# EMI-Group/evogp

Hardware: AMD Instinct MI355X
Metric: tree_evals_per_s (higher is better)
Workload: dtype f32; 1 GPU; BASELINE north_star / configs[2] shape: SymbolicRegression synthetic 10-var, GLOBAL pop=1000000 x 1024 datapoints, max_tree_len=64, funcs + - * /, one tree_SR_fitness pass over every rank's shard per step; global_pop=1000000, pop_per_gpu=1000000, datapoints=1024, var_len=10, max_tree_len=64, ranks=1, device_prewarm_calls=40

## Files before the change

### evogp_amd/_lib.py

```python
from __future__ import annotations

import ctypes as C
import os

_HERE = os.path.dirname(os.path.abspath(__file__))
LIB_PATH = os.environ.get("EVOGP_HIP_LIB") or os.path.join(_HERE, "lib", "libevogp_hip.so")

ABI_VERSION = 9

_vp = C.c_void_p
_u = C.c_uint
_i = C.c_int
_f = C.c_float

PROTOTYPES = {
    "evogp_hip_generate": [_u, _u, _u, _u, _u, _f, _f, _vp, _vp, _vp, _vp, _vp, _vp, _vp, _u, _vp],
    "evogp_hip_mutate": [_i, _i, _vp, _vp, _vp, _vp, _vp, _vp, _vp, _vp, _vp, _vp, _vp],
    "evogp_hip_crossover": [_i, _i, _i, _vp, _vp, _vp, _vp, _vp, _vp, _vp, _vp, _vp, _vp, _vp],
    "evogp_hip_evaluate": [_u, _u, _u, _u, _vp, _vp, _vp, _vp, _vp, _vp],
    "evogp_hip_sr_fitness": [_u, _u, _u, _u, _u, _i, _vp, _vp, _vp, _vp, _vp, _vp, _u, _vp],
    "evogp_hip_generate_masked": [_u, _u, _u, _u, _u, _f, _f, _vp, _vp, _vp, _vp, _vp, _vp, _vp, _u, _vp, _u, _vp],
    "evogp_hip_breed_default": [_i, _i, _i, _i, _vp, _vp, _vp, _vp, _vp, _u, _vp, _vp, _vp, _vp, _vp, _vp, _vp, _vp],
    "evogp_hip_breed_default_rows": [_i, _i, _i, _i, _vp, _vp, _vp, _vp, _vp, _u, _vp, _vp, _vp, _vp, _vp, _vp, _vp, _i, _i, _vp],
    "evogp_hip_breed_default_table": [_i, _i, _i, _i, _i, _vp, _vp, _vp, _vp, _vp, _u, _vp, _vp, _vp, _vp, _vp, _vp, _vp, _i, _i, _vp],
    "evogp_hip_breed_lists": [_i, _i, _i, _i, _i, _vp, _vp, _vp, _vp, _vp, _vp, _u, _vp, _vp, _vp, _vp, _vp, _vp, _vp, _i, _i, _vp],
    "evogp_hip_generate_masked_hashed": [_u, _u, _u, _u, _u, _f, _f, _vp, _vp, _vp, _vp, _vp, _vp, _u, C.c_longlong, C.c_longlong, _u, _vp],
    "evogp_hip_breed_lists_hashed": [_i, _i, _i, _i, _i, _vp, _vp, _vp, _vp, _vp, C.c_longlong, C.c_longlong, _u, _vp, _vp, _vp, _vp, _vp, _vp, _vp, _i, _i, _vp],
    "evogp_hip_sr_fitness_hinted": [_u, _u, _u, _u, _u, _i, _vp, _vp, _vp, _vp, _vp, _vp, _u, _u, _vp],
    "evogp_hip_batch_evaluate": [_u, _u, _u, _u, _u, _vp, _vp, _vp, _vp, _vp, _vp],
    "evogp_hip_batch_argmax_count": [_u, _u, _u, _u, _u, _vp, _vp, _vp, _vp, _vp, _vp, _vp],
    "evogp_hip_evaluate_prepare": [_u, _u, _u, _u, _vp, _vp, _vp, _vp, C.c_size_t, _vp],
    "evogp_hip_evaluate_prepared": [_u, _u, _u, _u, _vp, _vp, _vp, _vp, _i, _vp, _vp, _vp],
    "evogp_hip_structural_mutate": [_i, _i, _i, _f, _i, _i, _i, C.c_longlong, C.c_longlong, _vp, _vp, _vp, _vp, _vp, _vp, _vp, _vp],
    "evogp_hip_insert_mutate": [_i, _i, C.c_uint, _i, C.c_longlong, C.c_longlong, _vp, _vp, _vp, _vp, _vp, _vp, _vp, _vp, _vp, _vp, _vp],
    "evogp_hip_point_mutate": [_i, _i, _i, _f, _f, _i, _i, _i, _i, _i, _i, _i, C.c_longlong, C.c_longlong, _vp, _vp, _vp, _vp, _vp, _vp, _vp, _vp, _vp],
    "evogp_hip_random_words": [C.c_longlong, C.c_longlong, _i, C.c_longlong, C.c_longlong, C.c_longlong, _vp, _vp],
    "evogp_hip_fitness_scores": [_u, _i, _vp, _vp, _vp],
    "evogp_hip_select": [_u, _u, _u, _vp, _vp, _vp, _vp],
    "evogp_hip_select_alternating": [_u, _u, _u, _vp, _vp, _vp, _vp, _vp],
    "evogp_hip_tournament_select": [_u, _u, _u, C.c_longlong, C.c_longlong, _vp, _vp, _vp],
    "evogp_hip_set_program_buffer_limit": [C.c_ulonglong],
    "evogp_hip_release_workspaces": [],
    "evogp_hip_set_allocator": [_vp, _vp],
    "evogp_hip_set_sr_division": [C.c_int],
    "evogp_hip_get_sr_division": [],
    "evogp_hip_abi_version": [],
    "evogp_hip_sr_gradient": [_u, _u, _u, _u, _u, _i, _vp, _vp, _vp, _vp, _vp, _vp, _vp, _vp],
    "evogp_hip_sr_const_step": [_u, _u, _u, _i, _vp, _vp, _vp, _vp, _vp, _vp, _vp, _vp, _vp, _vp],
    "evogp_hip_sr_case_errors": [_u, _u, _u, _u, _u, _i, _vp, _vp, _vp, _vp, _vp, _vp, _vp],
    "evogp_hip_lexicase_workspace_bytes": [_u, _u, _u, C.POINTER(C.c_ulonglong)],
    "evogp_hip_lexicase_select": [_u, _u, _vp, _vp, _u, C.c_longlong, C.c_longlong, _vp, _vp, _vp],
    "evogp_hip_pareto_rank_workspace_bytes": [_u, C.POINTER(C.c_ulonglong)],
    "evogp_hip_pareto_rank": [_u, _u, _vp, _vp, _vp, _vp, _vp, _vp, _vp],
    "evogp_hip_nsga2_select": [_u, _vp, _u, _u, _u, C.c_longlong, C.c_longlong, _vp, _vp],
    "evogp_hip_sr_subtree_errors": [_u, _u, _u, _u, _u, _i, _vp, _vp, _vp, _vp, _vp, _vp, _vp, _vp],
    "evogp_hip_prune_rows": [_u, _u, _u, _i, _i, _vp, _vp, _vp, _vp, _vp, _vp, _vp, _vp, _vp, _vp, _vp],
}

DEBUG_PROTOTYPES = {
    "evogp_hip_timer_begin": [_vp],
    "evogp_hip_timer_end": [_vp, C.POINTER(C.c_float)],
    "evogp_hip_debug_set_stats": [_vp],
    "evogp_hip_debug_compile_batch": [_i],
    "evogp_hip_debug_long_compiler": [_i],
    "evogp_hip_debug_twins": [_i],
    "evogp_hip_debug_tc_fold": [_i],
    "evogp_hip_debug_profile": [_i],
    "evogp_hip_debug_profile_read": [C.POINTER(C.c_float), C.POINTER(C.c_int)],
    "evogp_hip_debug_tc_histogram": [_u, _vp, _i, _vp],
    "evogp_hip_debug_tc_nhandlers": [],
    "evogp_hip_debug_tc_program": [_u, _vp, _i],
    "evogp_hip_debug_forget_function_classes": [],
    "evogp_hip_debug_structural_mutate_given": [_i, _i, _i, _i, _i, _vp, _vp, _vp, _vp, _vp, _vp, _vp, _vp],
    "evogp_hip_debug_insert_mutate_given": [_i, _i, _i, _vp, _vp, _vp, _vp, _vp, _vp, _vp, _vp, _vp, _vp, _vp],
    "evogp_hip_debug_point_mutate_given": [_i, _i, _i, _i, _i, _i, _i, _i, _i, _vp, _vp, _vp, _vp, _vp, _vp, _vp, _vp, _vp, _vp, _vp, _vp, _vp, _vp],
    "evogp_hip_debug_lexicase": [_vp, _i],
    "evogp_hip_debug_pareto_rank": [_i],
}


def _load() -> C.CDLL:
    if not os.path.exists(LIB_PATH):
        raise ImportError(
            f"{LIB_PATH} is missing: build the HIP engine first "
            "(python -c 'import __graft_entry__ as g; g.build()'  or  make -C evogp_amd/csrc). "
            "evogp_amd has no CPU fallback."
        )
    lib = C.CDLL(LIB_PATH)
    for name, argtypes in list(PROTOTYPES.items()) + list(DEBUG_PROTOTYPES.items()):
        fn = getattr(lib, name)
        fn.argtypes = argtypes
        fn.restype = _i
    lib.evogp_hip_evaluate_workspace_bytes.argtypes = [_u, _u]
    lib.evogp_hip_evaluate_workspace_bytes.restype = C.c_size_t
    lib.evogp_hip_select_workspace_bytes.argtypes = []
    lib.evogp_hip_select_workspace_bytes.restype = C.c_size_t
    lib.evogp_hip_program_buffer_bytes.argtypes = []
    lib.evogp_hip_program_buffer_bytes.restype = C.c_ulonglong
    lib.evogp_hip_record_ring_bytes.argtypes = []
    lib.evogp_hip_record_ring_bytes.restype = C.c_ulonglong
    lib.evogp_hip_error_string.argtypes = [_i]
    lib.evogp_hip_error_string.restype = C.c_char_p
    got = lib.evogp_hip_abi_version()
    if got != ABI_VERSION:
        raise ImportError(f"libevogp_hip.so ABI version {got}, expected {ABI_VERSION}: rebuild the engine")
    return lib


lib = _load()


def check(code: int, what: str) -> None:
    if code != 0:
        raise RuntimeError(f"{what} failed: {lib.evogp_hip_error_string(code).decode()} (code {code})")
```

### evogp_amd/csrc/sr_tc.hip

```cpp
#include "interp.hpp"
#include "launch.hpp"
#include "sr_params.hpp"
#include "tc_interp_k8.inc"
#include "tc_interp_k4.inc"
#include "tc_interp_k1.inc"

#include <atomic>
#include <cstddef>
#include <mutex>
#include <cstdio>
#include <vector>

namespace evogp {

struct TcCompileParams {
    const float *value;
    const int16_t *type;
    const int16_t *size;
    uint2 *prog;
    float *fitness;
    unsigned *marks;
    unsigned *zero_next;
    int pop, gp_len, var_len;
    uint32_t unary_mask;
    uint32_t var_stride;
    uint32_t ydelta;
    uint32_t rec;
    uint32_t overflow;
    int depth;
    int out_len;
    int nblocks;
    int rows;
    int general;
    int heavy_reserve;
    int div_reserve;
    int classify;
    uint32_t recip;
    int twins;
    int long_fast;
    int learn;
    int nan_trees;
};

__device__ inline uint32_t division_in_place(uint32_t id, int after, const TcCompileParams &p) {
    if (id < 24u || id >= 32u) return id;
    const uint32_t form = id - 24u;
    const uint32_t ip = form == 0u ? (uint32_t)EVOGP_TC_H_DIVIP_SS : form == 3u ? (uint32_t)EVOGP_TC_H_DIVIP_SC : form == 4u ? (uint32_t)EVOGP_TC_H_DIVIP_CS : 0u;
    if (ip == 0u) return id;
    const int before = after + (form == 0u ? 1 : 0);
    return before + p.div_reserve <= p.depth ? ip : id;
}

enum : int { TC_S = 0, TC_V = 1, TC_C = 2 };
constexpr int kMarkSampleBlocks = 64;
constexpr int kZeroRounds = 3;
static std::atomic<int> g_long_fast{-1};
static std::atomic<int> g_twins{-1};
static std::atomic<int> g_fold{-1};
static std::atomic<int> g_compile_batch{-2};
static int tc_nan_trees() {
    static const int env_fold = env_int("EVOGP_TC_FOLD", 2);
    const int fo = g_fold.load(std::memory_order_relaxed);
    return fo >= 0 ? fo : (env_fold < 0 || env_fold > 2 ? 2 : env_fold);
}
static_assert(kSentinelHeavy == 0x7FC0FEEDu, "gen/gen_tc_asm.py SENTINEL_HEAVY");

__device__ inline float fold_bin4_fast(int op, float x, float y) {
    return op == 0 ? x + y : op == 1 ? x - y : op == 2 ? x * y : (y == 0.0f ? __builtin_nanf("") : x / y);
}

__device__ inline uint32_t tc_word0(int id, int slot, uint32_t pf_bytes, uint32_t aux = 0u) {
    return ((pf_bytes >> 10) << 24) | ((aux & 0xFFu) << 16) | (uint32_t)(((slot & 1) * EVOGP_TC_NHANDLERS + id) * EVOGP_TC_SLOT);
}

static_assert(EVOGP_TC_H_PUSH_V == EVOGP_TC_H_PUSH_C + 1 && EVOGP_TC_H_DIVIP_CS == EVOGP_TC_H_DIVIP_SS + 2 && EVOGP_TC_H_DIVR_CV == EVOGP_TC_H_DIVR_SV + 2 &&
              EVOGP_TC_H_PUSH_C_NP == EVOGP_TC_H_ADD_SS_NP + 24 && EVOGP_TC_H_DIVIP_SS_NP == EVOGP_TC_H_ADD_SS_NP + 26 &&
              EVOGP_TC_H_DIVR_SV_NP == EVOGP_TC_H_ADD_SS_NP + 29, "gen/gen_tc_asm.py NOPF_TWINS");
__device__ inline int no_prefetch_delta(bool arith3, bool push_c, bool in_place, bool by_recip) {
    return arith3 ? (int)EVOGP_TC_H_ADD_SS_NP : push_c ? (int)EVOGP_TC_H_PUSH_C_NP - (int)EVOGP_TC_H_PUSH_C
         : in_place ? (int)EVOGP_TC_H_DIVIP_SS_NP - (int)EVOGP_TC_H_DIVIP_SS : by_recip ? (int)EVOGP_TC_H_DIVR_SV_NP - (int)EVOGP_TC_H_DIVR_SV : 0;
}
__device__ inline bool next_word_has_variable(const TcCompileParams &, unsigned long long keptwave, bool kept, bool uses_var, bool is_root) {
    const unsigned long long U = __ballot(kept & uses_var);
    return __builtin_amdgcn_inverse_ballot_w64((((~keptwave) + (U << 1)) & keptwave) | __ballot(is_root));
}

__device__ inline void division_by_reciprocal(const TcCompileParams &p, int &id, uint32_t pf, uint32_t d1, uint32_t &aux) {
    const bool sv = id == 3 * 8 + 1, vv = id == 3 * 8 + 5, cv = id == 3 * 8 + 7;
    const bool ok = (p.recip != 0u) & (sv | vv | cv);
    const uint32_t voff = vv ? d1 << 4 : pf;
    aux = ok ? (voff + p.recip) >> 10 : aux;
    id = ok ? (int)EVOGP_TC_H_DIVR_SV + (int)vv + 2 * (int)cv : id;
}

constexpr int kUnaryInv = 10;
constexpr int kUnaryZero = 11;
__device__ __attribute__((always_inline)) inline float fold_unary_body(int op, float x) {
    switch (op) {
    case 0: return -x;
    case 1: return fabsf(x);
    case 2: return sinf(x);
    case 3: return cosf(x);
    case 4: return tanf(x);
    case 5: return sqrtf(x);
    case 6: return sqrtf(fabsf(x));
    case 7: return expf(x);
    case 8: return logf(x);
    case 9: return x == 0.0f ? -kMaxVal : logf(fabsf(x));
    case kUnaryZero: return 0.0f;
    default: return x == 0.0f ? __builtin_nanf("") : 1.0f / x;
    }
}
__device__ __attribute__((noinline)) float fold_unary(int op, float x) { return fold_unary_body(op, x); }

template <bool UN>
__device__ inline int compile_tree(const TcCompileParams &p, uint2 *rec, int len, int ty, int sz, float val, int lane) {
// ... 334 lines not shown
            int z = seli(L(Z0), 1, 0);
            int zr = bperm(z, ri4);
#pragma unroll
            for (int r = 0; r < kZeroRounds; ++r) {
                z |= (next(z) & ((zr & zboth) | zleft)) | (zr & zright);
                zr = bperm(z, ri4);
            }
            Mnan |= Mfn & Mop3 & B(zr != 0);
        }
    }
    const int nanincl = (int)__builtin_amdgcn_mbcnt_hi((uint32_t)(Mnan >> 32), __builtin_amdgcn_mbcnt_lo((uint32_t)Mnan, 0u)) + seli(L(Mnan), 1, 0);
    const int both = (int)((uint32_t)inclf << 15) | (nanincl << 8) | above;
    const int at_end = bperm(both, (end - 1) << 2), before = bperm(both, (lo - 1) << 2);
    const int base = seli(lo > 0, before >> 15, 0);
    const int slot = above - (at_end & 0xFF);
    const int totf = (at_end >> 15) - base;
    const int hf = seli(L(Mkept), totf - (inclf - base - deltaf), 0);
    M Mpz = Min & B(((at_end >> 8) & 127) != seli(lo > 0, (before >> 8) & 127, 0));
    if (U0 && Mpz != 0ull) {
        const M segmask = L(Min) ? ((len >= 64 ? ~0ull : ((1ull << len) - 1ull)) << lo) : 0ull;
        Mpz &= B((MU & segmask) == 0ull);
    }
    const M Mhigh = B(hf > p.depth);
    M Mlong = 0ull;
    if (U0) Mlong = Mroot & B(slot + 1 > 31);
    int cls = TREE_OK;
    if ((Min & (~(Mleaf | M4) | Msb | Mhigh | Mlong)) != 0ull) {
        const M segmask = L(Min) ? ((len >= 64 ? ~0ull : ((1ull << len) - 1ull)) << lo) : 0ull;
        auto seg_any = [&](M m) -> bool { return (m & segmask) != 0ull; };
        cls = seg_any(Min & B(kind == 3)) ? TREE_HEAVY : seg_any(Min & B(kind == 5)) ? TREE_GENERAL : seg_any(Min & Msb) ? TREE_HEAVY
            : seg_any(Min & Mhigh) ? (p.gp_len > 64 && p.general ? TREE_GENERAL : TREE_HEAVY) : seg_any(Mlong) ? TREE_HEAVY : TREE_OK;
    }
    const M Mdivown = MB & ~Mpushc & ~Mdivr & B(opx == 3);
    const M Mss = Mdivown & B(form == 0), Msc = Mdivown & B(form == 3), Mcs = Mdivown & B(form == 4);
    const int ip = seli(L(Mss), (int)EVOGP_TC_H_DIVIP_SS, seli(L(Msc), (int)EVOGP_TC_H_DIVIP_SC, (int)EVOGP_TC_H_DIVIP_CS));
    const M Minpl = (Mss | Msc | Mcs) & B(hf + seli(L(Mss), 1, 0) + p.div_reserve <= p.depth);
    id = seli(L(Minpl), ip, id);
    if (p.twins) {
        const M Muses = ~Mpushc & ~MU & ((MB & (MlV | MrV)) | (~MB & MV));
        const M Uk = Mkept & Muses;
        const M nxt = (((~keptwave) + (Uk << 1)) & keptwave) | Mroot;
        id += seli(L(nxt), 0, no_prefetch_delta(L(MB & ~Mpushc & ~Mdivr & B(opx < 3)), L(Mpushc), L(Minpl), L(Mdivr & ~Mpushc)));
    }
    const M Mok = B(cls == TREE_OK);
    if (L(Mkept & Mok & ~Mpz)) *(uint2 *)(rec0 + (roff + (uint32_t)slot * 8u)) = make_uint2(tc_word0(id, slot, pf, aux), d1);
    if (L(Mroot)) {
        uint32_t skip = tc_word0(EVOGP_TC_H_SKIP, 0, 0u), nan_tree = tc_word0(EVOGP_TC_H_NAN_TREE, 0, 0u);
        asm volatile("" : "+v"(skip), "+v"(nan_tree));
        const uint32_t last = selu(L(Mpz), nan_tree, tc_word0(EVOGP_TC_H_END, slot + 1, p.ydelta));
        *(uint2 *)(rec0 + (roff + (uint32_t)seli(L(Mok & ~Mpz), slot + 1, 0) * 8u)) = make_uint2(selu(L(Mok), last, skip), 0u);
    }
    if (cls == TREE_GENERAL && !p.general) cls = TREE_HEAVY;
    return L(Min) ? cls : (int)TREE_OK;
}

template <bool U0>
__device__ inline int compile_pack_arith_plain(const TcCompileParams &p, char *rec0, uint32_t roff, bool in, int lo, int len, int ty, int sz, float val, int lane) {
    auto bperm = [](int v, int i4) -> int { return __builtin_amdgcn_ds_bpermute(i4, v); };
    auto next = [](int v) -> int { return __builtin_amdgcn_update_dpp(0, v, 0x130 , 0xf, 0xf, true); };
    auto any = [](bool c) -> bool { return __builtin_amdgcn_ballot_w64(c) != 0ull; };
    auto seli = [](bool c, int x, int y) -> int { return c ? x : y; };
    auto selu = [](bool c, uint32_t x, uint32_t y) -> uint32_t { return c ? x : y; };
    auto self = [](bool c, float x, float y) -> float { return c ? x : y; };
    const int end = lo + len;
    const uint32_t f = (uint32_t)val;
    const bool isV = ty == T_VAR, isC = ty == T_CONST, isBf = ty == T_BFUNC;
    const uint32_t opu = f - (uint32_t)F_ADD;
    const bool is4 = isBf & (opu < 4u);
    const bool g5 = (isBf & (f - (uint32_t)F_LOOSE_DIV <= (uint32_t)(F_GE - F_LOOSE_DIV))) | (ty == T_TFUNC) | (ty == T_UFUNC);
    const int v = max(0, min((int)val, p.var_len - 1));
    const uint32_t pay = selu(isV, (uint32_t)v * p.var_stride, f2bits(val));
    const bool u0 = U0 && in & (ty == T_UFUNC) & (f - (uint32_t)F_SIN > (uint32_t)(F_LOOSE_SQRT - F_SIN)) & (p.unary_mask != 0u);
    const int kind = seli(isV, 0, seli(isC, 1, seli(is4, 2, seli(u0, 4, seli(g5, 5, 3)))));
    const int op = (int)(opu & 3u);
    const bool isB = in & (kind == 2), isU = U0 && u0;
    const int ks = kind | (sz << 3);
    const int ksl = next(ks);
    const int szl = ksl >> 3;
    const int ri = lane + 1 + szl, ri4 = ri << 2;
    const int ksr = bperm(ks, ri4);
    const int szr = ksr >> 3;
    const bool size_bad = (sz != seli(isB, 1 + szl + szr, seli(isU, 1 + szl, 1))) | (isB & ((szl < 1) | (ri >= end))) | (isU & ((szl < 1) | (lane + 1 >= end)));
    int kl = ksl & 7, kr = ksr & 7;
    uint32_t pl = (uint32_t)next((int)pay), pr = (uint32_t)bperm((int)pay, ri4);
    auto fold = [&](uint32_t a, uint32_t b, bool who) -> uint32_t {
        const float x = bits2f(a), y = bits2f(b);
        const float fa = x + y, fs = x - y, fm = x * y;
        float fd = fm;
        if (any(who & (op == 3))) fd = self(y == 0.0f, __builtin_nanf(""), x / y);
        return f2bits(self(op == 0, fa, self(op == 1, fs, self(op == 2, fm, fd))));
    };
    const bool absorbedB = isB & (kl == 1) & (kr == 1);
    const bool absorbed = absorbedB | (isU & (kl == 1));
    uint32_t folded = 0u;
    if (any(absorbed)) {
        folded = selu(absorbedB, fold(pl, pr, absorbedB), 0u);
        const int ek = seli(absorbed, 1, kind);
        const uint32_t ep = selu(absorbed, folded, pay);
        kl = next(ek); kr = bperm(ek, ri4);
        pl = (uint32_t)next((int)ep); pr = (uint32_t)bperm((int)ep, ri4);
    }
    if (U0) { kl = seli(kl == 4, 2, kl); kr = seli(kr == 4, 2, kr); }
    const bool cc = isB & !absorbed & (kl == 1) & (kr == 1);
    uint32_t folded2 = 0u;
    if (any(cc)) folded2 = fold(pl, pr, cc);
    const uint32_t cb = pr & 0x7FFFFFFFu, ex = cb >> 23;
// ... 1045 lines not shown
        else if (len <= 64) {
            if (__any(lane < len && ty == T_UFUNC && p.unary_mask != 0u)) cls = compile_tree<true>(p, rec, len, ty, sz, val, lane);
            else cls = compile_tree_arith(p, rec, len, ty, sz, val, lane);
        }
        if (cls == TREE_GENERAL && !p.general) cls = TREE_HEAVY;
        if (cls != TREE_OK && lane == 0) {
            rec[0] = make_uint2(tc_word0(EVOGP_TC_H_SKIP, 0, 0u), 0u);
            p.fitness[t] = cls == TREE_BAD ? __builtin_nanf("") : bits2f(cls == TREE_GENERAL ? kSentinelGeneral : kSentinelHeavy);
            if (cls == TREE_GENERAL && p.marks) p.marks[4] = 1u;
            else if (cls == TREE_HEAVY && p.marks) {
                p.marks[0] = 1u;
                if (blockIdx.x < kMarkSampleBlocks) atomicAdd(p.marks + 2, 1u);
            }
        }
    }
}

__device__ inline bool generic_node(int ty, float val) {
    const uint32_t f = (uint32_t)val;
    return (ty == T_TFUNC) | ((ty == T_BFUNC) & (f - (uint32_t)F_ADD >= 4u)) | ((ty == T_UFUNC) & ((f == (uint32_t)F_LOOSE_INV) | (f - (uint32_t)F_SINH <= 2u)));
}

template <int B, int MODE, bool LONGROWS>
__global__ __launch_bounds__(256) void tc_compile_packed_kernel(TcCompileParams p) {
    constexpr bool UN = MODE != 0;
    const int lane = threadIdx.x & 63;
    if (p.zero_next && blockIdx.x == 0)
        for (int i = threadIdx.x; i < kCallScratchWords; i += blockDim.x) p.zero_next[i] = 0u;
    const uint32_t wave_id = uni((blockIdx.x * blockDim.x + threadIdx.x) >> 6);
    const uint32_t t0 = wave_id * (uint32_t)B;
    if (t0 >= (uint32_t)p.pop) return;
    const int nb = (int)min((uint32_t)B, (uint32_t)p.pop - t0);
    const int L = p.gp_len;
    int raw = 1;
    if (lane < nb) raw = (int)p.size[(size_t)(t0 + (uint32_t)lane) * L];
    char *const rec0 = (char *)p.prog + (size_t)t0 * p.rec;
    const bool longer = LONGROWS && lane < nb && min(raw, L) > 64;
    if (LONGROWS && longer) {
        uint32_t skip = tc_word0(EVOGP_TC_H_SKIP, 0, 0u);
        asm volatile("" : "+v"(skip));
        *(uint2 *)(rec0 + (uint32_t)__mul24(lane, (int)p.rec)) = make_uint2(skip, 0u);
        p.fitness[t0 + (uint32_t)lane] = bits2f(p.general ? kSentinelGeneral : kSentinelHeavy);
        if (p.marks) {
            if (p.general) {
                const int n = min(raw, L);
                p.marks[p.long_fast ? 8 + (int)(n > 128) + (int)(n > 256) + (int)(n > 512) : 4] = 1u;
            }
            else {
                p.marks[0] = 1u;
                if ((wave_id >> 2) < (uint32_t)kMarkSampleBlocks) atomicAdd(p.marks + 2, 1u);
            }
        }
    }
    const int lens = lane < nb && !longer ? max(1, min(raw, L)) : 0;
    int sval = lens | (raw <= 0 ? 128 : 0) | (lane << 8);
#pragma unroll
    for (int r = 3; r < 7; ++r) {
        const unsigned long long ones = __builtin_amdgcn_ballot_w64((sval & (1 << r)) != 0);
        const int below1 = (int)__builtin_amdgcn_mbcnt_hi((uint32_t)(ones >> 32), __builtin_amdgcn_mbcnt_lo((uint32_t)ones, 0u));
        const int to = (sval & (1 << r)) ? below1 : __popcll(ones) + lane - below1;
        sval = __builtin_amdgcn_ds_permute(to << 2, sval);
    }
    const int slen = sval & 127;
    const size_t node0 = (size_t)t0 * (uint32_t)L;
    const float *const value0 = p.value + node0;
    const int16_t *const type0 = p.type + node0, *const size0 = p.size + node0;
    unsigned long long left = LONGROWS ? __builtin_amdgcn_ballot_w64(slen > 0) : (nb >= 64 ? ~0ull : (1ull << nb) - 1ull);
    bool n_in = false;
    unsigned long long n_inm = 0ull;
    int n_tb = 0, n_lo = 0, n_len = 0, n_bad = 0, n_ty = T_CONST, n_sz = 1;
    float n_val = 0.0f;
    auto plan = [&]() {
        int used = 0, about = 0;
        while (true) {
            const unsigned long long cand = __builtin_amdgcn_ballot_w64(slen <= 64 - used) & left;
            if (cand == 0ull) break;
            const int j = __builtin_ctzll(cand);
            left &= ~(1ull << j);
            const int sv = __builtin_amdgcn_readlane(sval, j), l = sv & 127;
            about = (uint32_t)(lane - used) < (uint32_t)l ? (sv | (used << 16)) : about;
            used += l;
            if (used >= 64) break;
        }
        n_in = lane < used;
        n_inm = used >= 64 ? ~0ull : (1ull << used) - 1ull;
        n_tb = (about >> 8) & 255; n_lo = about >> 16; n_len = about & 127; n_bad = about & 128;
        n_ty = T_CONST; n_sz = 1; n_val = 0.0f;
        if (n_in) {
            const uint32_t at = (uint32_t)(__mul24(n_tb, L) + lane - n_lo);
            n_ty = (int)*(const int16_t *)((const char *)type0 + at * 2u); n_val = *(const float *)((const char *)value0 + at * 4u);
            n_sz = (int)*(const int16_t *)((const char *)size0 + at * 2u);
        }
    };
    bool more = left != 0ull;
    if (more) plan();
    uint32_t seen = 0u;
    while (more) {
        const bool in = n_in;
        const unsigned long long inm = n_inm;
        const int tb = n_tb, lo = n_lo, len = n_len, bad = n_bad, sz = n_sz;
        const int ty = bad ? -1 : n_ty;
        const float val = n_val;
        more = left != 0ull;
        if (more) plan();
        const uint32_t roff = (uint32_t)__mul24(tb, (int)p.rec);
        int cls;
        const bool unary = __builtin_amdgcn_ballot_w64(ty == T_UFUNC) != 0ull;
        if (MODE == 3) cls = compile_pack_mo(p, rec0, roff, in, lo, len, ty, sz, val, lane);
        else if (MODE == 2 && __builtin_amdgcn_ballot_w64(generic_node(ty, val)) != 0ull) cls = compile_pack_generic(p, rec0, roff, in, lo, len, ty, sz, val, lane);
        else if (UN && unary && p.unary_mask != 0u) cls = compile_pack_unary<true>(p, rec0, roff, in, lo, len, ty, sz, val, lane);
        else if (!UN && unary) cls = compile_pack_arith<true>(p, rec0, roff, inm, lo, len, ty, sz, val, lane);
        else cls = compile_pack_arith<false>(p, rec0, roff, inm, lo, len, ty, sz, val, lane);
        if (MODE != 3 && p.learn) {
            const bool look = MODE != 0 || __builtin_amdgcn_ballot_w64(cls != TREE_OK) != 0ull;
            if (look) {
                const bool gen = __builtin_amdgcn_ballot_w64(generic_node(ty, val)) != 0ull;
                const bool un = unary && __builtin_amdgcn_ballot_w64((ty == T_UFUNC) & ((uint32_t)val - (uint32_t)F_SIN <= (uint32_t)(F_LOOSE_SQRT - F_SIN))) != 0ull;
                seen |= ((un | gen) ? 1u : 0u) | (gen ? 2u : 0u);
            }
        }
        if (cls != TREE_OK && in && lane == lo) {
            const bool nan = bad != 0 || cls == TREE_BAD;
            p.fitness[t0 + (uint32_t)tb] = nan ? __builtin_nanf("") : bits2f(cls == TREE_GENERAL ? kSentinelGeneral : kSentinelHeavy);
            if (!nan && p.marks) {
                if (cls == TREE_GENERAL) p.marks[p.long_fast ? 8 : 4] = 1u;
                else {
                    p.marks[0] = 1u;
                    if ((wave_id >> 2) < (uint32_t)kMarkSampleBlocks) atomicAdd(p.marks + 2, 1u);
                }
            }
        }
    }
    if (MODE != 3 && p.learn && p.marks && uni((int)seen) != 0 && lane == 0) {
        p.marks[5] = 1u;
        if (seen & 2u) p.marks[6] = 1u;
    }
}


__device__ __attribute__((always_inline)) inline int compile_long_arith(const TcCompileParams &p, char *rec0, int t, int len, char *lds, int lane,
                                                           int ty0, float val0, int sz0, int ty1, float val1, int sz1, int lds_len) {
    auto any = [](bool c) -> bool { return __builtin_amdgcn_ballot_w64(c) != 0ull; };
    auto seli = [](bool c, int x, int y) -> int { return c ? x : y; };
    auto selu = [](bool c, uint32_t x, uint32_t y) -> uint32_t { return c ? x : y; };
    const int L = lds_len;
    uint32_t *ks_s = (uint32_t *)lds;
// ... 886 lines not shown
        }
        records = (char *)d.prog;
    }
    if (!d.last_use && (e = hipEventCreateWithFlags(&d.last_use, hipEventDisableTiming)) != hipSuccess) return e;
    d.last_pop = p.pop; d.last_rec = rec; d.last_overflow = (uint32_t)overflow;

    int chunks = 1;
    static const int env_chunks = env_int("EVOGP_TC_CHUNKS", 0);
    if (p.marks && !capturing && !STATS && !p.prof_mid && pieces == 1) {
        if (env_chunks > 0) chunks = env_chunks;
        if (chunks > kCallScratchChunks) chunks = kCallScratchChunks;
        if (chunks > 1 && p.pop / chunks < 20000) chunks = p.pop / 20000 > 0 ? p.pop / 20000 : 1;
    }
    if (chunks > 1) {
        if (!d.side && (e = hipStreamCreateWithFlags(&d.side, hipStreamNonBlocking)) != hipSuccess) return e;
        if (!d.fork && (e = hipEventCreateWithFlags(&d.fork, hipEventDisableTiming)) != hipSuccess) return e;
        for (int i = 0; i < chunks; ++i)
            if (!d.ready[i] && (e = hipEventCreateWithFlags(&d.ready[i], hipEventDisableTiming)) != hipSuccess) return e;
        if (wg_waves * 2 > waves_per_cu) wg_waves = waves_per_cu / 2 > 0 ? waves_per_cu / 2 : 1;
        wgs_per_cu = 1;
    }
    *mark_sample = 0;
    static const int env_general = env_int("EVOGP_TC_GENERAL", 1);
    static const int env_unary = env_int("EVOGP_TC_UNARY", EVOGP_TC_UNARY_MASK | (1 << kUnaryInv));
    static const int env_cblocks = env_int("EVOGP_TC_CBLOCKS", 0);
    static const int env_divip = env_int("EVOGP_TC_DIVIP", 1);
    static const int env_long_fast = env_int("EVOGP_TC_LONG_FAST", 1);
    if (p.out_len > 1 && env_general == 0) return hipSuccess;

    auto compile_params = [&](int lo, int n, unsigned *marks, bool first) -> TcCompileParams {
        TcCompileParams c{};
        c.value = p.value + (size_t)lo * p.gp_len; c.type = p.type + (size_t)lo * p.gp_len; c.size = p.size + (size_t)lo * p.gp_len;
        c.prog = (uint2 *)(records + (size_t)lo * rec); c.fitness = p.fitness + lo; c.marks = marks;
        c.zero_next = first ? p.zero_next : nullptr;
        c.pop = n; c.gp_len = p.gp_len; c.var_len = p.var_len;
        c.var_stride = (uint32_t)(tiles * G * 1024);
        c.ydelta = c.var_stride * (uint32_t)p.var_len;
        c.rec = rec; c.depth = DEPTH; c.overflow = (uint32_t)overflow;
        c.out_len = p.out_len; c.nblocks = nblocks; c.rows = K;
        c.heavy_reserve = (EVOGP_TC_HEAVY_REGS + K - 1) / K;
        c.div_reserve = env_divip ? (EVOGP_TC_DIVIP_REGS + K - 1) / K : 1 << 20;
        c.classify = p.classify;
        c.recip = recip ? (uint32_t)(p.var_len + label_cols) * c.var_stride : 0u;
        {
            static const int env_twins = env_int("EVOGP_TC_TWINS", 1);
            const int tw = g_twins.load(std::memory_order_relaxed);
            c.twins = tw >= 0 ? tw : (env_twins == 2 || (env_twins == 1 && (long)n >= 900l * info.num_cus));
        }
        c.general = env_general != 0;
        { const int lf = g_long_fast.load(std::memory_order_relaxed); c.long_fast = (lf >= 0 ? lf : env_long_fast) && p.out_len == 1 && p.gp_len >= 128 && c.general; }
        c.unary_mask = (uint32_t)env_unary & ((uint32_t)EVOGP_TC_UNARY_MASK | (1u << kUnaryInv));
        c.learn = p.feedback != nullptr && marks != nullptr;
        c.nan_trees = tc_nan_trees();
        return c;
    };
    bool learn_packed = false;
    auto launch_marked_general = [&](const TcCompileParams &c, int n, hipStream_t strm) {
        long gblocks = ((long)n + 63) / 64;
        if (gblocks > (long)info.num_cus * 16) gblocks = (long)info.num_cus * 16;
        if (p.gp_len <= 64) { hipLaunchKernelGGL(tc_compile_general_kernel<false>, dim3((unsigned)gblocks), dim3(256), 0, strm, c, 0, 0, p.gp_len); return; }
        if (c.long_fast && c.general && c.gp_len >= 128) {
            if (4 * tc_long_lds_bytes(c.gp_len) > 64 * 1024 && !d.attr_set[16]) {
                (void)hipFuncSetAttribute((const void *)tc_compile_long_kernel, hipFuncAttributeMaxDynamicSharedMemorySize, 160 * 1024 - 1024);
                (void)hipGetLastError();
                d.attr_set[16] = true;
            }
            int lo_len = 0, klass = 0;
            for (int hi_len = 128; ; hi_len *= 2, ++klass) {
                if (hi_len > c.gp_len) hi_len = c.gp_len;
                const int group = hi_len <= 256 ? 16 : 64;
                hipLaunchKernelGGL(tc_compile_long_kernel, dim3((unsigned)((n + group - 1) / group)), dim3(256), 4 * tc_long_lds_bytes(hi_len), strm, c, lo_len, hi_len, group, klass);
                if (hi_len >= c.gp_len) break;
                lo_len = hi_len;
            }
        }
        hipLaunchKernelGGL(tc_compile_general_kernel<true>, dim3((unsigned)gblocks), dim3(256), 4 * tc_general_lds_bytes(p.gp_len), strm, c, 0, 0, p.gp_len);
    };
    auto launch_compilers = [&](int lo, int n, unsigned *marks, bool first, hipStream_t strm) -> hipError_t {
        const TcCompileParams c = compile_params(lo, n, marks, first);
        long cblocks = ((long)n + 3) / 4;
        long cmax = (long)info.num_cus * 32;
        if (env_cblocks > 0) cmax = env_cblocks;
        if (cblocks > cmax) cblocks = cmax;
        if (first) {
            const long nwaves = cblocks * 4, sw = kMarkSampleBlocks * 4 < nwaves ? kMarkSampleBlocks * 4 : nwaves;
            long sample = 0;
            for (long w = 0; w < sw && w < n; ++w) sample += (n - 1 - w) / nwaves + 1;
            *mark_sample = (int)sample;
        }
        const size_t clds = 4 * tc_general_lds_bytes(p.gp_len);
        if (clds > 64 * 1024 && !d.attr_set[15]) {
            (void)hipFuncSetAttribute((const void *)tc_compile_general_kernel<true>, hipFuncAttributeMaxDynamicSharedMemorySize, 160 * 1024 - 1024);
            (void)hipGetLastError();
            d.attr_set[15] = true;
        }
        static const int env_packed_env = env_int("EVOGP_TC_PACKED", -1);
        const int set_packed = g_compile_batch.load(std::memory_order_relaxed);
        const int env_packed = set_packed != -2 ? set_packed : env_packed_env;
        static const int env_generic = env_int("EVOGP_TC_PACK_GENERIC", 1);
        const bool packed_mo = p.out_len > 1 && env_packed != 0 && env_generic != 0;
        const bool packed = (p.out_len == 1 && env_packed != 0) || packed_mo;
        if (packed) {
            const bool un = c.nblocks != 1;
            constexpr unsigned kOwnHandlers = (1u << F_ADD) | (1u << F_SUB) | (1u << F_MUL) | (1u << F_DIV) | (1u << F_SIN) | (1u << F_COS) | (1u << F_TAN) |
                                              (1u << F_LOG) | (1u << F_LOOSE_LOG) | (1u << F_EXP) | (1u << F_INV) | (1u << F_NEG) | (1u << F_ABS) |
                                              (1u << F_SQRT) | (1u << F_LOOSE_SQRT);
// ... 439 lines not shown
    if (p.out_len > 1 && p.out_len + 3 > EVOGP_TC_K8_DEPTH && k == 8) {
        if (env_wide && p.out_len + 3 <= EVOGP_TC_K8W_DEPTH && !p.stats) wide = true; else k = 4;
    }
    if (p.out_len > 1 && p.out_len + 3 > EVOGP_TC_K4_DEPTH && k == 4) return hipSuccess;
    if (p.out_len > 1 && p.out_len + 3 > EVOGP_TC_K1_DEPTH) return hipSuccess;
    static const int env_k = env_int("EVOGP_TC_K", 0);
    if (env_k == 1 || env_k == 4 || env_k == 8) k = env_k;
#ifndef EVOGP_FUSED_STATS
    if (p.stats) return run_tc<8, true>(p, stream, handled, mark_sample, mark_chunks);
#endif
    const int dm = sr_division_mode();
#ifdef EVOGP_FUSED_STATS
    static const int env_fused = env_int("EVOGP_TC_FUSED", 1);
#else
    static const int env_fused = env_int("EVOGP_TC_FUSED", -1);
#endif
    const bool fused_ok = k == 8 && p.out_len == 1 && !p.classify && p.gp_len <= 64 && p.marks && !p.prof_mid;
    auto fused = [&]() -> hipError_t {
        return dm == 1 ? run_fused<1>(p, stream, handled, mark_sample, mark_chunks)
             : dm == 2 ? run_fused<2>(p, stream, handled, mark_sample, mark_chunks)
                       : run_fused<0>(p, stream, handled, mark_sample, mark_chunks);
    };
    if (env_fused == 1 && fused_ok && !p.hint_general) {
        hipError_t fe = fused();
        if (fe != hipSuccess || *handled) return fe;
    }
#define EVOGP_RUN_TC(F) (wide && k == 8 ? run_tc<8, false, F, true>(p, stream, handled, mark_sample, mark_chunks) \
                        : k == 8 ? run_tc<8, false, F>(p, stream, handled, mark_sample, mark_chunks) \
                        : k == 4 ? run_tc<4, false, F>(p, stream, handled, mark_sample, mark_chunks) \
                                 : run_tc<1, false, F>(p, stream, handled, mark_sample, mark_chunks))
    hipError_t te = dm == 1 ? EVOGP_RUN_TC(1) : dm == 2 ? EVOGP_RUN_TC(2) : EVOGP_RUN_TC(0);
#undef EVOGP_RUN_TC
    if (te == hipSuccess && *handled && env_fused != 0 && fused_ok) fused_keep_spare(stream);
    if (te != hipSuccess || *handled || env_fused == 0 || !fused_ok) return te;
    if (g_prog_limit.load(std::memory_order_relaxed) == 0ull) return te;
    *mark_sample = 0; *mark_chunks = 1;
    return fused();
}

}

extern "C" int evogp_hip_debug_twins(int mode) {
    if (mode < -1 || mode > 1) return EVOGP_E_BADARG;
    evogp::g_twins.store(mode, std::memory_order_relaxed);
    return EVOGP_OK;
}

extern "C" int evogp_hip_debug_tc_fold(int mode) {
    if (mode < -1 || mode > 2) return EVOGP_E_BADARG;
    evogp::g_fold.store(mode, std::memory_order_relaxed);
    return EVOGP_OK;
}

extern "C" int evogp_hip_debug_long_compiler(int fast) {
    if (fast < -1 || fast > 1) return EVOGP_E_BADARG;
    evogp::g_long_fast.store(fast, std::memory_order_relaxed);
    return EVOGP_OK;
}

extern "C" int evogp_hip_debug_compile_batch(int trees) {
    if (trees < -1 || trees > 64) return EVOGP_E_BADARG;
    evogp::g_compile_batch.store(trees, std::memory_order_relaxed);
    return EVOGP_OK;
}

extern "C" int evogp_hip_set_program_buffer_limit(unsigned long long bytes) {
    evogp::g_prog_limit.store(bytes, std::memory_order_relaxed);
    return EVOGP_OK;
}

extern "C" int evogp_hip_set_allocator(evogp_alloc_fn alloc, evogp_free_fn free_fn) {
    if ((alloc == nullptr) != (free_fn == nullptr)) return EVOGP_E_BADARG;
    for (auto &d : evogp::g_tc) {
        std::lock_guard<std::mutex> lock(d.mu);
        if (d.prog || d.graph_prog || !d.retired.empty() || !d.rings.empty() || d.spare_ring) return EVOGP_E_BADARG;
    }
    if (evogp::grad_workspaces_held() || evogp::case_workspaces_held()) return EVOGP_E_BADARG;
    evogp::g_alloc.store(alloc, std::memory_order_release);
    evogp::g_free.store(free_fn, std::memory_order_release);
    return EVOGP_OK;
}

extern "C" unsigned long long evogp_hip_program_buffer_bytes(void) {
    int dev = 0;
    (void)hipGetDevice(&dev);
    evogp::TcDevice &d = evogp::g_tc[dev & 63];
    std::lock_guard<std::mutex> lock(d.mu);
    return (unsigned long long)(d.prog_bytes + d.graph_bytes + d.retired_bytes);
}

extern "C" unsigned long long evogp_hip_record_ring_bytes(void) {
    int dev = 0;
    (void)hipGetDevice(&dev);
    evogp::TcDevice &d = evogp::g_tc[dev & 63];
    std::lock_guard<std::mutex> lock(d.mu);
    return (unsigned long long)(d.ring_bytes * (d.rings.size() + (d.spare_ring ? 1u : 0u)));
}

extern "C" int evogp_hip_debug_forget_function_classes(void) {
    int dev = 0;
    (void)hipGetDevice(&dev);
    evogp::TcDevice &d = evogp::g_tc[dev & 63];
    std::lock_guard<std::mutex> lock(d.mu);
    for (auto &k : d.fb_key) k = {};
    return EVOGP_OK;
}
// ... 57 lines not shown
```

### include/evogp_hip_debug.h

```cpp
#ifndef EVOGP_HIP_DEBUG_H
#define EVOGP_HIP_DEBUG_H
#include "evogp_hip.h"
#ifdef __cplusplus
extern "C" {
#endif

int evogp_hip_timer_begin(evogp_stream_t stream);
int evogp_hip_timer_end(evogp_stream_t stream, float *elapsed_ms);

int evogp_hip_debug_set_stats(unsigned long long *device_counters);

int evogp_hip_debug_profile(int enable);
int evogp_hip_debug_profile_read(float *stage_ms , int *calls);

int evogp_hip_debug_compile_batch(int trees);
int evogp_hip_debug_long_compiler(int fast);
int evogp_hip_debug_twins(int mode);
int evogp_hip_debug_tc_fold(int mode);

int evogp_hip_debug_tc_histogram(unsigned pop, unsigned long long *device_hist, int hist_len, evogp_stream_t stream);
int evogp_hip_debug_tc_nhandlers(void);
int evogp_hip_debug_tc_program(unsigned tree, unsigned *host_words, int max_words);

int evogp_hip_debug_forget_function_classes(void);

int evogp_hip_debug_structural_mutate_given(int pop_size, int gp_len, int mode, int inner_is_offset, int skip_rows, const int *given,
                                            const float *value, const int16_t *type, const int16_t *size, float *value_res,
                                            int16_t *type_res, int16_t *size_res, evogp_stream_t stream);
int evogp_hip_debug_insert_mutate_given(int pop_size, int gp_len, int skip_rows, const int *given, const float *value, const int16_t *type,
                                        const int16_t *size, const float *donor_value, const int16_t *donor_type, const int16_t *donor_size,
                                        float *value_res, int16_t *type_res, int16_t *size_res, evogp_stream_t stream);
int evogp_hip_debug_point_mutate_given(int pop_size, int gp_len, int mode, int modify_output, int fix_roulette, int skip_rows, int input_len,
                                       int output_len, int n_consts, const unsigned char *target, const float *u, const int *var_idx,
                                       const int *const_idx, const int *out_idx, const float *value, const int16_t *type, const int16_t *size,
                                       const float *roulette_ufuncs, const float *roulette_bfuncs, const float *roulette_tfuncs,
                                       const float *const_samples, float *value_res, evogp_stream_t stream);

int evogp_hip_debug_lexicase(unsigned long long *device_counters, int stop_after);

int evogp_hip_debug_pareto_rank(int stop_after);

#ifdef __cplusplus
}
#endif
#endif
```

Before: 1680 billion tree-evals/s.

## Pre-screen trees for guaranteed NaN before compile and skip their compilation

Adds a wave-level screening pass in the tree compiler that packs tree rows into the wavefront in groups of four. It checks structurally, using ballots, DPP and bpermute, whether an arithmetic tree contains an overflowing constant or a division by a zero constant with valid structure and depth. Trees that are certain to evaluate to NaN get a NaN-tree record written directly and their length zeroed, so the sort and compile stages skip them. The pass is on by default through EVOGP_TC_SCREEN whenever NaN-tree folding is enabled. It adds an extra pass over every tree row, which costs work on populations where few trees are screened out.

```diff
diff --git a/evogp_amd/_lib.py b/evogp_amd/_lib.py
--- a/evogp_amd/_lib.py
+++ b/evogp_amd/_lib.py
@@ -65,6 +65,7 @@
     "evogp_hip_debug_long_compiler": [_i],
     "evogp_hip_debug_twins": [_i],
     "evogp_hip_debug_tc_fold": [_i],
+    "evogp_hip_debug_tc_screen": [_i],
     "evogp_hip_debug_profile": [_i],
     "evogp_hip_debug_profile_read": [C.POINTER(C.c_float), C.POINTER(C.c_int)],
     "evogp_hip_debug_tc_histogram": [_u, _vp, _i, _vp],
diff --git a/evogp_amd/csrc/sr_tc.hip b/evogp_amd/csrc/sr_tc.hip
--- a/evogp_amd/csrc/sr_tc.hip
+++ b/evogp_amd/csrc/sr_tc.hip
@@ -40,6 +40,7 @@
     int long_fast;
     int learn;
     int nan_trees;
+    int screen;
 };
 
 __device__ inline uint32_t division_in_place(uint32_t id, int after, const TcCompileParams &p) {
@@ -57,11 +58,17 @@
 static std::atomic<int> g_long_fast{-1};
 static std::atomic<int> g_twins{-1};
 static std::atomic<int> g_fold{-1};
+static std::atomic<int> g_screen{-1};
 static std::atomic<int> g_compile_batch{-2};
 static int tc_nan_trees() {
     static const int env_fold = env_int("EVOGP_TC_FOLD", 2);
     const int fo = g_fold.load(std::memory_order_relaxed);
     return fo >= 0 ? fo : (env_fold < 0 || env_fold > 2 ? 2 : env_fold);
+}
+static int tc_screen() {
+    static const int env_screen = env_int("EVOGP_TC_SCREEN", 1);
+    const int sc = g_screen.load(std::memory_order_relaxed);
+    return sc >= 0 ? sc : (env_screen != 0);
 }
 static_assert(kSentinelHeavy == 0x7FC0FEEDu, "gen/gen_tc_asm.py SENTINEL_HEAVY");
 
@@ -502,6 +509,45 @@
     }
     if (cls == TREE_GENERAL && !p.general) cls = TREE_HEAVY;
     return L(Min) ? cls : (int)TREE_OK;
+}
+
+__device__ inline unsigned long long screen_pack_arith(const TcCompileParams &p, unsigned long long inm, int lo, int len, int ty, int sz, float val, int lane) {
+    typedef unsigned long long M;
+    auto bperm = [](int v, int i4) -> int { return __builtin_amdgcn_ds_bpermute(i4, v); };
+    auto next = [](int v) -> int { return __builtin_amdgcn_update_dpp(0, v, 0x130 , 0xf, 0xf, true); };
+    auto B = [](bool c) -> M { return __builtin_amdgcn_ballot_w64(c); };
+    auto L = [](M m) -> bool { return __builtin_amdgcn_inverse_ballot_w64(m); };
+    auto seli = [](bool c, int x, int y) -> int { return c ? x : y; };
+    const M Min = inm;
+    const int end = lo + len;
+    const uint32_t opu = (uint32_t)val - (uint32_t)F_ADD;
+    const uint32_t mag2 = f2bits(val) << 1;
+    const M MC = B(ty == T_CONST);
+    const M M4 = B(ty == T_BFUNC) & B(opu < 4u);
+    const M MB = Min & M4;
+    const int w = (sz << 1) | seli(L(MC & B(mag2 == 0u)), 1, 0);
+    const int szl = next(w) >> 1;
+    const int ri = lane + 1 + szl;
+    const int wr = bperm(w, ri << 2);
+    const int szr = wr >> 1;
+    const M Msb = B(sz != seli(L(MB), 1 + szl + szr, 1)) | (MB & (B(szl < 1) | B(ri >= end)));
+    const M Mhit = Min & ((MC & B(mag2 > 0xFF000000u)) | (MB & B(opu == 3u) & B((wr & 1) != 0)));
+    if (Mhit == 0ull) return 0ull;
+    M Mout = Min & (~(B(ty == T_VAR) | MC | M4) | Msb);
+    const int delta = seli(L(MB), (int)(szl == 1) + (int)(szr == 1) - 1, 0);
+    const int incl = wave_scan_incl(delta);
+    const int hitincl = (int)__builtin_amdgcn_mbcnt_hi((uint32_t)(Mhit >> 32), __builtin_amdgcn_mbcnt_lo((uint32_t)Mhit, 0u)) + seli(L(Mhit), 1, 0);
+    const int both = (int)((uint32_t)incl << 8) | hitincl;
+    const int at_end = bperm(both, (end - 1) << 2), before = bperm(both, (lo - 1) << 2);
+    const int base = seli(lo > 0, before >> 8, 0);
+    const int height = ((at_end >> 8) - base) - (incl - base - delta);
+    Mout |= Min & B(height > p.depth);
+    M Mtake = Min & B(lane == lo) & B(((at_end & 127) != seli(lo > 0, before & 127, 0)));
+    if (Mout != 0ull) {
+        const M segmask = L(Min) ? ((len >= 64 ? ~0ull : ((1ull << len) - 1ull)) << lo) : 0ull;
+        Mtake &= B((Mout & segmask) == 0ull);
+    }
+    return Mtake;
 }
 
 template <bool U0>
@@ -1653,26 +1699,20 @@
             }
         }
     }
-    const int lens = lane < nb && !longer ? max(1, min(raw, L)) : 0;
+    int lens = lane < nb && !longer ? max(1, min(raw, L)) : 0;
     int sval = lens | (raw <= 0 ? 128 : 0) | (lane << 8);
-#pragma unroll
-    for (int r = 3; r < 7; ++r) {
-        const unsigned long long ones = __builtin_amdgcn_ballot_w64((sval & (1 << r)) != 0);
-        const int below1 = (int)__builtin_amdgcn_mbcnt_hi((uint32_t)(ones >> 32), __builtin_amdgcn_mbcnt_lo((uint32_t)ones, 0u));
-        const int to = (sval & (1 << r)) ? below1 : __popcll(ones) + lane - below1;
-        sval = __builtin_amdgcn_ds_permute(to << 2, sval);
-    }
-    const int slen = sval & 127;
+    int slen = lens;
     const size_t node0 = (size_t)t0 * (uint32_t)L;
     const float *const value0 = p.value + node0;
     const int16_t *const type0 = p.type + node0, *const size0 = p.size + node0;
-    unsigned long long left = LONGROWS ? __builtin_amdgcn_ballot_w64(slen > 0) : (nb >= 64 ? ~0ull : (1ull << nb) - 1ull);
+    unsigned long long left = 0ull;
     bool n_in = false;
     unsigned long long n_inm = 0ull;
     int n_tb = 0, n_lo = 0, n_len = 0, n_bad = 0, n_ty = T_CONST, n_sz = 1;
     float n_val = 0.0f;
-    auto plan = [&]() {
-        int used = 0, about = 0;
+    auto share_out = [&](int &about) -> int {
+        int used = 0;
+        about = 0;
         while (true) {
             const unsigned long long cand = __builtin_amdgcn_ballot_w64(slen <= 64 - used) & left;
             if (cand == 0ull) break;
@@ -1683,6 +1723,11 @@
             used += l;
             if (used >= 64) break;
         }
+        return used;
+    };
+    auto plan = [&]() {
+        int about;
+        const int used = share_out(about);
         n_in = lane < used;
         n_inm = used >= 64 ? ~0ull : (1ull << used) - 1ull;
         n_tb = (about >> 8) & 255; n_lo = about >> 16; n_len = about & 127; n_bad = about & 128;
@@ -1693,6 +1738,60 @@
             n_sz = (int)*(const int16_t *)((const char *)size0 + at * 2u);
         }
     };
+    auto plan_screen = [&](unsigned long long &o_inm, int &o_about, int &o_ty, int &o_sz, float &o_val) {
+        const int used = share_out(o_about);
+        o_inm = used >= 64 ? ~0ull : (1ull << used) - 1ull;
+        const uint32_t at = lane < used ? (uint32_t)(__mul24((o_about >> 8) & 255, L) + lane - (o_about >> 16)) : 0u;
+        o_ty = (int)*(const int16_t *)((const char *)type0 + at * 2u); o_val = *(const float *)((const char *)value0 + at * 4u);
+        o_sz = (int)*(const int16_t *)((const char *)size0 + at * 2u);
+    };
+    if (MODE == 0 && !LONGROWS && p.screen) {
+        constexpr int kScreenGroup = 4;
+        left = __builtin_amdgcn_ballot_w64(lane < nb && raw > 0);
+        unsigned long long screened = 0ull;
+        unsigned long long q_inm[kScreenGroup];
+        int q_about[kScreenGroup], q_ty[kScreenGroup], q_sz[kScreenGroup];
+        float q_val[kScreenGroup];
+#pragma unroll
+        for (int k = 0; k < kScreenGroup; ++k) plan_screen(q_inm[k], q_about[k], q_ty[k], q_sz[k], q_val[k]);
+        while (q_inm[0] != 0ull) {
+            unsigned long long c_inm[kScreenGroup];
+            int c_about[kScreenGroup], c_ty[kScreenGroup], c_sz[kScreenGroup];
+            float c_val[kScreenGroup];
+#pragma unroll
+            for (int k = 0; k < kScreenGroup; ++k) { c_inm[k] = q_inm[k]; c_about[k] = q_about[k]; c_ty[k] = q_ty[k]; c_sz[k] = q_sz[k]; c_val[k] = q_val[k]; }
+#pragma unroll
+            for (int k = 0; k < kScreenGroup; ++k) plan_screen(q_inm[k], q_about[k], q_ty[k], q_sz[k], q_val[k]);
+#pragma unroll
+            for (int k = 0; k < kScreenGroup; ++k) {
+                if (c_inm[k] != 0ull) {
+                    const int tb = (c_about[k] >> 8) & 255, lo = c_about[k] >> 16, len = c_about[k] & 127;
+                    unsigned long long take = screen_pack_arith(p, c_inm[k], lo, len, c_ty[k], c_sz[k], c_val[k], lane);
+                    while (take != 0ull) {
+                        const int j = __builtin_ctzll(take);
+                        take &= take - 1ull;
+                        screened |= 1ull << __builtin_amdgcn_readlane(tb, j);
+                    }
+                }
+            }
+        }
+        if (__builtin_amdgcn_inverse_ballot_w64(screened)) {
+            uint32_t nan_tree = tc_word0(EVOGP_TC_H_NAN_TREE, 0, 0u);
+            asm volatile("" : "+v"(nan_tree));
+            *(uint2 *)(rec0 + (uint32_t)__mul24(lane, (int)p.rec)) = make_uint2(nan_tree, 0u);
+            lens = 0;
+        }
+        sval = lens | (raw <= 0 ? 128 : 0) | (lane << 8);
+    }
+#pragma unroll
+    for (int r = 3; r < 7; ++r) {
+        const unsigned long long ones = __builtin_amdgcn_ballot_w64((sval & (1 << r)) != 0);
+        const int below1 = (int)__builtin_amdgcn_mbcnt_hi((uint32_t)(ones >> 32), __builtin_amdgcn_mbcnt_lo((uint32_t)ones, 0u));
+        const int to = (sval & (1 << r)) ? below1 : __popcll(ones) + lane - below1;
+        sval = __builtin_amdgcn_ds_permute(to << 2, sval);
+    }
+    slen = sval & 127;
+    left = __builtin_amdgcn_ballot_w64(slen > 0);
     bool more = left != 0ull;
     if (more) plan();
     uint32_t seen = 0u;
@@ -2685,6 +2784,7 @@
         c.unary_mask = (uint32_t)env_unary & ((uint32_t)EVOGP_TC_UNARY_MASK | (1u << kUnaryInv));
         c.learn = p.feedback != nullptr && marks != nullptr;
         c.nan_trees = tc_nan_trees();
+        c.screen = c.nan_trees != 0 && tc_screen() != 0;
         return c;
     };
     bool learn_packed = false;
@@ -3230,6 +3330,12 @@
     return EVOGP_OK;
 }
 
+extern "C" int evogp_hip_debug_tc_screen(int mode) {
+    if (mode < -1 || mode > 1) return EVOGP_E_BADARG;
+    evogp::g_screen.store(mode, std::memory_order_relaxed);
+    return EVOGP_OK;
+}
+
 extern "C" int evogp_hip_debug_long_compiler(int fast) {
     if (fast < -1 || fast > 1) return EVOGP_E_BADARG;
     evogp::g_long_fast.store(fast, std::memory_order_relaxed);
diff --git a/include/evogp_hip_debug.h b/include/evogp_hip_debug.h
--- a/include/evogp_hip_debug.h
+++ b/include/evogp_hip_debug.h
@@ -17,6 +17,7 @@
 int evogp_hip_debug_long_compiler(int fast);
 int evogp_hip_debug_twins(int mode);
 int evogp_hip_debug_tc_fold(int mode);
+int evogp_hip_debug_tc_screen(int mode);
 
 int evogp_hip_debug_tc_histogram(unsigned pop, unsigned long long *device_hist, int hist_len, evogp_stream_t stream);
 int evogp_hip_debug_tc_nhandlers(void);
```

Result: no change. 1674 billion tree-evals/s (-0.3%).
